# marqo-ai/marqo

Measured on NVIDIA H100. Metric: embeddings/s (open_clip/ViT-L-14 image vectorise, batch 256 per GPU), higher is better.
Workload: dtype bf16

## Files before the change

marqo_b200/csrc/attention.cuh:

```cuda
#pragma once
#include <type_traits>

#include "common.cuh"

namespace mb {
namespace attention {

enum Mask { MASK_NONE = 0, MASK_CAUSAL = 1, MASK_KEYLEN = 2 };

constexpr int BQ = 64;

struct RelBias {
    const float* table = nullptr;
    int smax = 0;
};
constexpr int MAX_BIAS_S = 1024;

int launch(const __nv_bfloat16* qkv, __nv_bfloat16* out, int B, int S, int W, int H, int mask, const int32_t* kv_len,
           const RelBias& bias, cudaStream_t stream);

void launch_wgmma_kernel(const __nv_bfloat16* qkv, __nv_bfloat16* out, int B, int S, int W, int H, int hd, int mask,
                         const int32_t* kv_len, const RelBias& bias, cudaStream_t stream);

inline int head_dim(int W, int H) {
    if (H > 0 && W == H * 64) return 64;
    if (H > 0 && W == H * 32) return 32;
    fail(B200_ERR_UNSUPPORTED, "attention: head_dim must be 32 or 64 (width %d, heads %d)", W, H);
}

inline float head_scale_log2e(int hd) { return (hd == 64 ? 0.125f : 0.17677669529663687f) * 1.4426950408889634f; }

template <class F>
void dispatch(int hd, int mask, bool bias, F&& f) {
    if (bias) return f(std::integral_constant<int, 64>{}, std::integral_constant<int, MASK_KEYLEN>{}, std::true_type{});
    const auto with_mask = [&](auto d) {
        if (mask == MASK_NONE)
            f(d, std::integral_constant<int, MASK_NONE>{}, std::false_type{});
        else if (mask == MASK_CAUSAL)
            f(d, std::integral_constant<int, MASK_CAUSAL>{}, std::false_type{});
        else
            f(d, std::integral_constant<int, MASK_KEYLEN>{}, std::false_type{});
    };
    if (hd == 64)
        with_mask(std::integral_constant<int, 64>{});
    else
        with_mask(std::integral_constant<int, 32>{});
}

struct KeyRange {
    int len, nkb;
};
template <int MASK, int BKV>
__device__ __forceinline__ KeyRange key_range(int S, const int32_t* __restrict__ kv_len, int b, int q0) {
    int len = S;
    if (MASK == MASK_KEYLEN) len = min(S, max(kv_len[b], 0));
    int kend = len;
    if (MASK == MASK_CAUSAL) kend = min(len, q0 + BQ);
    return {len, (kend + BKV - 1) / BKV};
}

template <int BKV, int THREADS>
__device__ __forceinline__ void stage_bias_band(float* band, const float* __restrict__ rel_bias, int smax, int h, int q0,
                                                int nkb) {
    const float* row = rel_bias + (size_t)h * (2 * smax - 1);
    for (int t = threadIdx.x; t < nkb * BKV + BQ; t += THREADS) {
        const int idx = t - (q0 + BQ - 1) + smax - 1;
        band[t] = idx >= 0 && idx < 2 * smax - 1 ? __ldg(row + idx) : 0.f;
    }
}

template <int MASK, bool BIAS>
struct OnlineSoftmax {
    int qrow[2];
    int q0;
    int len;
    float scale_log2e;
    const float* band;
    float row_sum[2] = {0.f, 0.f};
    float row_max[2] = {-INFINITY, -INFINITY};

    template <int NS, int NO>
    __device__ __forceinline__ void update(float (&s)[NS], float (&o)[NO], uint32_t (&pa)[NS / 8][4], int key0) {
        const int t = threadIdx.x & 3;
        float mx[2] = {row_max[0], row_max[1]};
#pragma unroll
        for (int i = 0; i < NS / 4; ++i) {
#pragma unroll
            for (int e = 0; e < 4; ++e) {
                const int key = key0 + 8 * i + 2 * t + (e & 1);
                const int rr = e >> 1;
                bool ok = key < len;
                if (MASK == MASK_CAUSAL) ok = ok && key <= qrow[rr];
                float v;
                if constexpr (BIAS)
                    v = ok ? s[4 * i + e] * scale_log2e + band[key - qrow[rr] + (q0 + BQ - 1)] : -INFINITY;
                else
                    v = ok ? s[4 * i + e] * scale_log2e : -INFINITY;
                s[4 * i + e] = v;
                mx[rr] = fmaxf(mx[rr], v);
            }
        }
        float corr[2], msafe[2];
#pragma unroll
        for (int rr = 0; rr < 2; ++rr) {
            mx[rr] = fmaxf(mx[rr], __shfl_xor_sync(0xffffffffu, mx[rr], 1));
            mx[rr] = fmaxf(mx[rr], __shfl_xor_sync(0xffffffffu, mx[rr], 2));
            msafe[rr] = mx[rr] == -INFINITY ? 0.f : mx[rr];
            corr[rr] = exp2f(row_max[rr] - msafe[rr]);
            row_max[rr] = mx[rr];
            row_sum[rr] *= corr[rr];
        }
#pragma unroll
        for (int i = 0; i < NO / 4; ++i) {
            o[4 * i] *= corr[0];
            o[4 * i + 1] *= corr[0];
            o[4 * i + 2] *= corr[1];
            o[4 * i + 3] *= corr[1];
        }
#pragma unroll
        for (int i = 0; i < NS / 4; ++i) {
            const float p0 = exp2f(s[4 * i] - msafe[0]), p1 = exp2f(s[4 * i + 1] - msafe[0]);
            const float p2 = exp2f(s[4 * i + 2] - msafe[1]), p3 = exp2f(s[4 * i + 3] - msafe[1]);
            row_sum[0] += p0 + p1;
            row_sum[1] += p2 + p3;
            pa[i >> 1][(i & 1) * 2] = pack_bf16x2(p0, p1);
            pa[i >> 1][(i & 1) * 2 + 1] = pack_bf16x2(p2, p3);
        }
    }

    __device__ __forceinline__ void finish(float (&inv)[2]) {
#pragma unroll
        for (int rr = 0; rr < 2; ++rr) {
            row_sum[rr] += __shfl_xor_sync(0xffffffffu, row_sum[rr], 1);
            row_sum[rr] += __shfl_xor_sync(0xffffffffu, row_sum[rr], 2);
        }
        inv[0] = row_sum[0] > 0.f ? 1.f / row_sum[0] : 0.f;
        inv[1] = row_sum[1] > 0.f ? 1.f / row_sum[1] : 0.f;
    }
};

}
}
```

marqo_b200/csrc/attention_wgmma.cu:

```cuda
#include <mutex>

#include "attention.cuh"
#include "ptx.cuh"

namespace mb {
namespace attention {

namespace {

constexpr int BKV = 128;
constexpr int KV_STAGES = 2;
constexpr int THREADS = 160;

template <int HD>
struct Tiles {
    static constexpr uint32_t Q_BYTES = BQ * HD * 2;
    static constexpr uint32_t KV_TILE_BYTES = BKV * HD * 2;
    static constexpr uint32_t STAGE_BYTES = 2 * KV_TILE_BYTES;
    static constexpr size_t SMEM_BYTES = Q_BYTES + KV_STAGES * STAGE_BYTES + 1024  + 64 ;
};

template <int HD>
__device__ __forceinline__ uint64_t desc_k(uint32_t smem_addr) {
    if constexpr (HD == 64) return ptx::make_desc_k_sw128(smem_addr);
    else return ptx::make_desc_k_sw64(smem_addr);
}
template <int HD>
__device__ __forceinline__ uint64_t desc_mn(uint32_t smem_addr) {
    if constexpr (HD == 64) return ptx::make_desc_mn_sw128(smem_addr, 0);
    else return ptx::make_desc_mn_sw64(smem_addr, 0);
}

template <int HD>
__device__ __forceinline__ void wgmma_pv(float (&o)[HD / 2], const uint32_t (&a)[4], uint64_t desc_v) {
    if constexpr (HD == 64) ptx::wgmma_m64n64k16_bf16_rs_tb(o, a, desc_v, 1u);
    else ptx::wgmma_m64n32k16_bf16_rs_tb(o, a, desc_v, 1u);
}

inline size_t bias_band_bytes(int S) { return ((size_t)(S + BKV - 1) / BKV * BKV + BQ) * sizeof(float); }

template <int HD, int MASK, bool BIAS>
__global__ void __launch_bounds__(THREADS)
attention_wgmma_kernel(const __grid_constant__ CUtensorMap tmap_q, const __grid_constant__ CUtensorMap tmap_kv,
                       __nv_bfloat16* __restrict__ out, int S, int W, const int32_t* __restrict__ kv_len,
                       float scale_log2e, const float* __restrict__ rel_bias, int bias_smax) {
    constexpr uint32_t Q_BYTES = Tiles<HD>::Q_BYTES;
    constexpr uint32_t KV_TILE_BYTES = Tiles<HD>::KV_TILE_BYTES;
    constexpr uint32_t STAGE_BYTES = Tiles<HD>::STAGE_BYTES;
    extern __shared__ uint8_t smem_raw[];
    uint8_t* smem = reinterpret_cast<uint8_t*>((reinterpret_cast<uintptr_t>(smem_raw) + 1023) & ~uintptr_t(1023));
    uint8_t* sq = smem;
    uint8_t* skv = smem + Q_BYTES;
    uint64_t* full = reinterpret_cast<uint64_t*>(skv + KV_STAGES * STAGE_BYTES);
    uint64_t* empty = full + KV_STAGES;
    uint64_t* qfull = empty + KV_STAGES;

    const int b = blockIdx.z, h = blockIdx.y, q0 = blockIdx.x * BQ;
    const int warp = threadIdx.x >> 5, lane = threadIdx.x & 31;
    const KeyRange kr = key_range<MASK, BKV>(S, kv_len, b, q0);
    const int nkb = kr.nkb;
    const int row0 = b * S;

    if (threadIdx.x == 0) {
        for (int i = 0; i < KV_STAGES; ++i) {
            ptx::mbar_init(&full[i], 1);
            ptx::mbar_init(&empty[i], 4);
        }
        ptx::mbar_init(qfull, 1);
        ptx::fence_barrier_init();
    }
    float* sbias = reinterpret_cast<float*>(reinterpret_cast<uint8_t*>(full) + 64);
    if constexpr (BIAS) stage_bias_band<BKV, THREADS>(sbias, rel_bias, bias_smax, h, q0, nkb);
    __syncthreads();

    if (warp == 4) {
        if (lane == 0 && nkb > 0) {
            ptx::mbar_arrive_expect_tx(qfull, Q_BYTES);
            ptx::tma_load_2d(sq, &tmap_q, qfull, h * HD, row0 + q0, ptx::kEvictFirst);
            for (int j = 0; j < nkb; ++j) {
                const int st = j % KV_STAGES;
                ptx::mbar_wait(&empty[st], ((uint32_t)(j / KV_STAGES) & 1u) ^ 1u);
                ptx::mbar_arrive_expect_tx(&full[st], STAGE_BYTES);
                uint8_t* dst = skv + (size_t)st * STAGE_BYTES;
                ptx::tma_load_2d(dst, &tmap_kv, &full[st], W + h * HD, row0 + j * BKV, ptx::kEvictLast);
                ptx::tma_load_2d(dst + KV_TILE_BYTES, &tmap_kv, &full[st], 2 * W + h * HD, row0 + j * BKV, ptx::kEvictLast);
            }
        }
        return;
    }

    const int g = lane >> 2, t = lane & 3;
    float o[HD / 2];
#pragma unroll
    for (int i = 0; i < HD / 2; ++i) o[i] = 0.f;
    OnlineSoftmax<MASK, BIAS> sm{{q0 + warp * 16 + g, q0 + warp * 16 + g + 8}, q0, kr.len, scale_log2e, sbias};
    if (nkb > 0) ptx::mbar_wait(qfull, 0);
    const uint32_t q_base = ptx::smem_u32(sq);
    for (int j = 0; j < nkb; ++j) {
        const int st = j % KV_STAGES;
        ptx::mbar_wait(&full[st], (uint32_t)(j / KV_STAGES) & 1u);
        const uint32_t k_base = ptx::smem_u32(skv + (size_t)st * STAGE_BYTES);
        const uint32_t v_base = k_base + KV_TILE_BYTES;
        float s[BKV / 2];
        ptx::wgmma_fence();
#pragma unroll
        for (int k = 0; k < HD / 16; ++k)
            ptx::wgmma_m64n128k16_bf16(s, desc_k<HD>(q_base + k * 32), desc_k<HD>(k_base + k * 32), k != 0 ? 1u : 0u);
        ptx::wgmma_commit();
        ptx::wgmma_wait<0>();
        uint32_t pa[BKV / 16][4];
        sm.update(s, o, pa, j * BKV);
        ptx::wgmma_fence();
#pragma unroll
        for (int k = 0; k < BKV / 16; ++k) wgmma_pv<HD>(o, pa[k], desc_mn<HD>(v_base + k * 32 * HD));
        ptx::wgmma_commit();
        ptx::wgmma_wait<0>();
        __syncwarp();
        if (lane == 0) ptx::mbar_arrive(&empty[st]);
    }
    float inv[2];
    sm.finish(inv);
#pragma unroll
    for (int rr = 0; rr < 2; ++rr) {
        if (sm.qrow[rr] >= S) continue;
        __nv_bfloat16* dst = out + ((size_t)row0 + sm.qrow[rr]) * W + h * HD + 2 * t;
#pragma unroll
        for (int i = 0; i < HD / 8; ++i)
            *reinterpret_cast<uint32_t*>(dst + 8 * i) =
                pack_bf16x2(o[4 * i + 2 * rr] * inv[rr], o[4 * i + 2 * rr + 1] * inv[rr]);
    }
}

template <int HD>
void make_tmaps(const __nv_bfloat16* qkv, int B, int S, int W, CUtensorMap& tq, CUtensorMap& tkv) {
    const uint64_t rows = (uint64_t)B * S;
    const CUtensorMapSwizzle swz = HD == 64 ? CU_TENSOR_MAP_SWIZZLE_128B : CU_TENSOR_MAP_SWIZZLE_64B;
    tq = make_tmap_2d(qkv, CU_TENSOR_MAP_DATA_TYPE_BFLOAT16, 2, (uint64_t)3 * W, rows, (uint64_t)3 * W * 2, HD, BQ, swz);
    tkv = make_tmap_2d(qkv, CU_TENSOR_MAP_DATA_TYPE_BFLOAT16, 2, (uint64_t)3 * W, rows, (uint64_t)3 * W * 2, HD, BKV, swz);
}

}

void launch_wgmma_kernel(const __nv_bfloat16* qkv, __nv_bfloat16* out, int B, int S, int W, int H, int hd, int mask,
                         const int32_t* kv_len, const RelBias& bias, cudaStream_t stream) {
    dispatch(hd, mask, bias.table != nullptr, [&](auto d, auto m, auto with_bias) {
        constexpr int HD = decltype(d)::value, MASK = decltype(m)::value;
        constexpr bool BIAS = decltype(with_bias)::value;
        constexpr size_t BASE = Tiles<HD>::SMEM_BYTES;
        static std::once_flag once;
        std::call_once(once, [] {
            MB_CUDA(cudaFuncSetAttribute(attention_wgmma_kernel<HD, MASK, BIAS>,
                                         cudaFuncAttributeMaxDynamicSharedMemorySize,
                                         (int)(BASE + (BIAS ? bias_band_bytes(MAX_BIAS_S) : 0))));
        });
        CUtensorMap tq, tkv;
        make_tmaps<HD>(qkv, B, S, W, tq, tkv);
        attention_wgmma_kernel<HD, MASK, BIAS>
            <<<dim3((S + BQ - 1) / BQ, H, B), THREADS, BASE + (BIAS ? bias_band_bytes(S) : 0), stream>>>(
                tq, tkv, out, S, W, kv_len, head_scale_log2e(HD), bias.table, bias.smax);
    });
}

}
}
```

marqo_b200/csrc/ptx.cuh:

```cuda
#pragma once
#include <cstdint>
#include <cstdio>
#include <cuda.h>
#include <cuda_runtime.h>

namespace ptx {

__device__ __forceinline__ uint32_t smem_u32(const void* p) {
    return static_cast<uint32_t>(__cvta_generic_to_shared(p));
}

__device__ __forceinline__ void st_shared_u32(uint32_t addr, uint32_t v) {
    asm volatile("st.shared.b32 [%0], %1;" ::"r"(addr), "r"(v) : "memory");
}
__device__ __forceinline__ void st_shared_f32x2(uint32_t addr, float x, float y) {
    asm volatile("st.shared.v2.f32 [%0], {%1, %2};" ::"r"(addr), "f"(x), "f"(y) : "memory");
}
__device__ __forceinline__ uint32_t ld_shared_u32(uint32_t addr) {
    uint32_t v;
    asm volatile("ld.shared.b32 %0, [%1];" : "=r"(v) : "r"(addr) : "memory");
    return v;
}
__device__ __forceinline__ float2 ld_shared_f32x2(uint32_t addr) {
    float2 v;
    asm volatile("ld.shared.v2.f32 {%0, %1}, [%2];" : "=f"(v.x), "=f"(v.y) : "r"(addr) : "memory");
    return v;
}

__device__ __forceinline__ uint32_t lane_id() {
    uint32_t l;
    asm volatile("mov.u32 %0, %%laneid;" : "=r"(l));
    return l;
}

__device__ __forceinline__ uint64_t globaltimer_ns() {
    uint64_t t;
    asm volatile("mov.u64 %0, %%globaltimer;" : "=l"(t));
    return t;
}

__device__ __forceinline__ bool elect_one() {
    uint32_t pred;
    asm volatile(
        "{\n"
        ".reg .pred p;\n"
        "elect.sync _|p, 0xffffffff;\n"
        "selp.u32 %0, 1, 0, p;\n"
        "}\n"
        : "=r"(pred));
    return pred != 0;
}

__device__ __forceinline__ void mbar_init(uint64_t* bar, uint32_t count) {
    asm volatile("mbarrier.init.shared::cta.b64 [%0], %1;" ::"r"(smem_u32(bar)), "r"(count) : "memory");
}
__device__ __forceinline__ void fence_barrier_init() {
    asm volatile("fence.mbarrier_init.release.cluster;" ::: "memory");
}
__device__ __forceinline__ void fence_proxy_async_smem() {
    asm volatile("fence.proxy.async.shared::cta;" ::: "memory");
}
__device__ __forceinline__ void mbar_arrive_expect_tx(uint64_t* bar, uint32_t bytes) {
    asm volatile("mbarrier.arrive.expect_tx.shared::cta.b64 _, [%0], %1;" ::"r"(smem_u32(bar)), "r"(bytes)
                 : "memory");
}
__device__ __forceinline__ void mbar_arrive(uint64_t* bar) {
    asm volatile("mbarrier.arrive.shared::cta.b64 _, [%0];" ::"r"(smem_u32(bar)) : "memory");
}
__device__ __forceinline__ bool mbar_try_wait(uint64_t* bar, uint32_t parity) {
    uint32_t ok;
    asm volatile(
        "{\n"
        ".reg .pred p;\n"
        "mbarrier.try_wait.parity.shared::cta.b64 p, [%1], %2;\n"
        "selp.u32 %0, 1, 0, p;\n"
        "}\n"
        : "=r"(ok)
        : "r"(smem_u32(bar)), "r"(parity)
        : "memory");
    return ok != 0;
}
__device__ __forceinline__ void mbar_wait(uint64_t* bar, uint32_t parity) {
    if (mbar_try_wait(bar, parity)) return;
    uint64_t t0 = globaltimer_ns();
    uint32_t spins = 0;
    while (!mbar_try_wait(bar, parity)) {
        if ((++spins & 0x3ff) == 0 && globaltimer_ns() - t0 > 4000000000ull) __trap();
    }
}

constexpr uint64_t kEvictNormal = 0x1000000000000000ull;
constexpr uint64_t kEvictFirst = 0x12F0000000000000ull;
constexpr uint64_t kEvictLast = 0x14F0000000000000ull;

__device__ __forceinline__ void prefetch_tmap(const CUtensorMap* tmap) {
    asm volatile("prefetch.tensormap [%0];" ::"l"(reinterpret_cast<uint64_t>(tmap)) : "memory");
}

__device__ __forceinline__ void tma_load_2d(void* smem_dst, const CUtensorMap* tmap, uint64_t* bar, int32_t c0,
                                            int32_t c1, uint64_t cache_hint) {
    asm volatile(
        "cp.async.bulk.tensor.2d.shared::cluster.global.tile.mbarrier::complete_tx::bytes.L2::cache_hint"
        " [%0], [%1, {%3, %4}], [%2], %5;"
        ::"r"(smem_u32(smem_dst)), "l"(reinterpret_cast<uint64_t>(tmap)), "r"(smem_u32(bar)), "r"(c0), "r"(c1),
        "l"(cache_hint)
        : "memory");
}

__device__ __forceinline__ void tma_prefetch_l2_2d(const CUtensorMap* tmap, int32_t c0, int32_t c1) {
    asm volatile("cp.async.bulk.prefetch.tensor.2d.L2.global.tile [%0, {%1, %2}];" ::"l"(reinterpret_cast<uint64_t>(tmap)),
                 "r"(c0), "r"(c1)
                 : "memory");
}

__device__ __forceinline__ void tma_store_2d(const CUtensorMap* tmap, const void* smem_src, int32_t c0, int32_t c1) {
    asm volatile("cp.async.bulk.tensor.2d.global.shared::cta.tile.bulk_group [%0, {%2, %3}], [%1];" ::"l"(
                     reinterpret_cast<uint64_t>(tmap)),
                 "r"(smem_u32(smem_src)), "r"(c0), "r"(c1)
                 : "memory");
}
__device__ __forceinline__ void tma_store_commit() { asm volatile("cp.async.bulk.commit_group;" ::: "memory"); }
template <int N>
__device__ __forceinline__ void tma_store_wait_read() {
    asm volatile("cp.async.bulk.wait_group.read %0;" ::"n"(N) : "memory");
}
template <int N>
__device__ __forceinline__ void tma_store_wait() {
    asm volatile("cp.async.bulk.wait_group %0;" ::"n"(N) : "memory");
}

__device__ __forceinline__ uint64_t make_desc_k_sw128(uint32_t smem_addr) {
    uint64_t d = 0;
    d |= static_cast<uint64_t>((smem_addr & 0x3FFFF) >> 4);
    d |= static_cast<uint64_t>(1) << 16;
    d |= static_cast<uint64_t>(1024 >> 4) << 32;
    d |= static_cast<uint64_t>(1) << 62;
    return d;
}

__device__ __forceinline__ uint64_t make_desc_mn_sw128(uint32_t smem_addr, uint32_t lbo_bytes) {
    uint64_t d = 0;
    d |= static_cast<uint64_t>((smem_addr & 0x3FFFF) >> 4);
    d |= static_cast<uint64_t>((lbo_bytes >> 4) & 0x3FFF) << 16;
    d |= static_cast<uint64_t>(1024 >> 4) << 32;
    d |= static_cast<uint64_t>(1) << 62;
    return d;
}

__device__ __forceinline__ uint64_t make_desc_k_sw64(uint32_t smem_addr) {
    uint64_t d = 0;
    d |= static_cast<uint64_t>((smem_addr & 0x3FFFF) >> 4);
    d |= static_cast<uint64_t>(1) << 16;
    d |= static_cast<uint64_t>(512 >> 4) << 32;
    d |= static_cast<uint64_t>(2) << 62;
    return d;
}

__device__ __forceinline__ uint64_t make_desc_mn_sw64(uint32_t smem_addr, uint32_t lbo_bytes) {
    uint64_t d = 0;
    d |= static_cast<uint64_t>((smem_addr & 0x3FFFF) >> 4);
    d |= static_cast<uint64_t>((lbo_bytes >> 4) & 0x3FFF) << 16;
    d |= static_cast<uint64_t>(512 >> 4) << 32;
    d |= static_cast<uint64_t>(2) << 62;
    return d;
}

__device__ __forceinline__ void wgmma_fence() { asm volatile("wgmma.fence.sync.aligned;" ::: "memory"); }
__device__ __forceinline__ void wgmma_commit() { asm volatile("wgmma.commit_group.sync.aligned;" ::: "memory"); }
template <int N>
__device__ __forceinline__ void wgmma_wait() {
    asm volatile("wgmma.wait_group.sync.aligned %0;" ::"n"(N) : "memory");
}

__device__ __forceinline__ void wgmma_m64n128k16_f16(float (&d)[64], uint64_t desc_a, uint64_t desc_b, uint32_t scale_d) {
    asm volatile(
        "{\n"
        ".reg .pred p;\n"
        "setp.ne.b32 p, %66, 0;\n"
        "wgmma.mma_async.sync.aligned.m64n128k16.f32.f16.f16 "
        "{"
        "%0, %1, %2, %3, %4, %5, %6, %7, %8, %9, %10, %11, %12, %13, %14, %15, "
        "%16, %17, %18, %19, %20, %21, %22, %23, %24, %25, %26, %27, %28, %29, %30, %31, "
        "%32, %33, %34, %35, %36, %37, %38, %39, %40, %41, %42, %43, %44, %45, %46, %47, "
        "%48, %49, %50, %51, %52, %53, %54, %55, %56, %57, %58, %59, %60, %61, %62, %63"
        "}, %64, %65, p, 1, 1, 0, 0;\n"
        "}\n"
        : "+f"(d[0]), "+f"(d[1]), "+f"(d[2]), "+f"(d[3]), "+f"(d[4]), "+f"(d[5]), "+f"(d[6]), "+f"(d[7]),
          "+f"(d[8]), "+f"(d[9]), "+f"(d[10]), "+f"(d[11]), "+f"(d[12]), "+f"(d[13]), "+f"(d[14]), "+f"(d[15]),
          "+f"(d[16]), "+f"(d[17]), "+f"(d[18]), "+f"(d[19]), "+f"(d[20]), "+f"(d[21]), "+f"(d[22]), "+f"(d[23]),
          "+f"(d[24]), "+f"(d[25]), "+f"(d[26]), "+f"(d[27]), "+f"(d[28]), "+f"(d[29]), "+f"(d[30]), "+f"(d[31]),
          "+f"(d[32]), "+f"(d[33]), "+f"(d[34]), "+f"(d[35]), "+f"(d[36]), "+f"(d[37]), "+f"(d[38]), "+f"(d[39]),
          "+f"(d[40]), "+f"(d[41]), "+f"(d[42]), "+f"(d[43]), "+f"(d[44]), "+f"(d[45]), "+f"(d[46]), "+f"(d[47]),
          "+f"(d[48]), "+f"(d[49]), "+f"(d[50]), "+f"(d[51]), "+f"(d[52]), "+f"(d[53]), "+f"(d[54]), "+f"(d[55]),
          "+f"(d[56]), "+f"(d[57]), "+f"(d[58]), "+f"(d[59]), "+f"(d[60]), "+f"(d[61]), "+f"(d[62]), "+f"(d[63])
        : "l"(desc_a), "l"(desc_b), "r"(scale_d));
}
__device__ __forceinline__ void wgmma_m64n128k16_bf16(float (&d)[64], uint64_t desc_a, uint64_t desc_b, uint32_t scale_d) {
    asm volatile(
        "{\n"
        ".reg .pred p;\n"
        "setp.ne.b32 p, %66, 0;\n"
        "wgmma.mma_async.sync.aligned.m64n128k16.f32.bf16.bf16 "
        "{"
        "%0, %1, %2, %3, %4, %5, %6, %7, %8, %9, %10, %11, %12, %13, %14, %15, "
        "%16, %17, %18, %19, %20, %21, %22, %23, %24, %25, %26, %27, %28, %29, %30, %31, "
        "%32, %33, %34, %35, %36, %37, %38, %39, %40, %41, %42, %43, %44, %45, %46, %47, "
        "%48, %49, %50, %51, %52, %53, %54, %55, %56, %57, %58, %59, %60, %61, %62, %63"
        "}, %64, %65, p, 1, 1, 0, 0;\n"
        "}\n"
        : "+f"(d[0]), "+f"(d[1]), "+f"(d[2]), "+f"(d[3]), "+f"(d[4]), "+f"(d[5]), "+f"(d[6]), "+f"(d[7]),
          "+f"(d[8]), "+f"(d[9]), "+f"(d[10]), "+f"(d[11]), "+f"(d[12]), "+f"(d[13]), "+f"(d[14]), "+f"(d[15]),
          "+f"(d[16]), "+f"(d[17]), "+f"(d[18]), "+f"(d[19]), "+f"(d[20]), "+f"(d[21]), "+f"(d[22]), "+f"(d[23]),
          "+f"(d[24]), "+f"(d[25]), "+f"(d[26]), "+f"(d[27]), "+f"(d[28]), "+f"(d[29]), "+f"(d[30]), "+f"(d[31]),
          "+f"(d[32]), "+f"(d[33]), "+f"(d[34]), "+f"(d[35]), "+f"(d[36]), "+f"(d[37]), "+f"(d[38]), "+f"(d[39]),
          "+f"(d[40]), "+f"(d[41]), "+f"(d[42]), "+f"(d[43]), "+f"(d[44]), "+f"(d[45]), "+f"(d[46]), "+f"(d[47]),
          "+f"(d[48]), "+f"(d[49]), "+f"(d[50]), "+f"(d[51]), "+f"(d[52]), "+f"(d[53]), "+f"(d[54]), "+f"(d[55]),
          "+f"(d[56]), "+f"(d[57]), "+f"(d[58]), "+f"(d[59]), "+f"(d[60]), "+f"(d[61]), "+f"(d[62]), "+f"(d[63])
        : "l"(desc_a), "l"(desc_b), "r"(scale_d));
}
__device__ __forceinline__ void wgmma_m64n256k16_bf16(float (&d)[128], uint64_t desc_a, uint64_t desc_b, uint32_t scale_d) {
    asm volatile(
        "{\n"
        ".reg .pred p;\n"
        "setp.ne.b32 p, %130, 0;\n"
        "wgmma.mma_async.sync.aligned.m64n256k16.f32.bf16.bf16 "
        "{"
        "%0, %1, %2, %3, %4, %5, %6, %7, %8, %9, %10, %11, %12, %13, %14, %15, "
        "%16, %17, %18, %19, %20, %21, %22, %23, %24, %25, %26, %27, %28, %29, %30, %31, "
        "%32, %33, %34, %35, %36, %37, %38, %39, %40, %41, %42, %43, %44, %45, %46, %47, "
        "%48, %49, %50, %51, %52, %53, %54, %55, %56, %57, %58, %59, %60, %61, %62, %63, "
        "%64, %65, %66, %67, %68, %69, %70, %71, %72, %73, %74, %75, %76, %77, %78, %79, "
        "%80, %81, %82, %83, %84, %85, %86, %87, %88, %89, %90, %91, %92, %93, %94, %95, "
        "%96, %97, %98, %99, %100, %101, %102, %103, %104, %105, %106, %107, %108, %109, %110, %111, "
        "%112, %113, %114, %115, %116, %117, %118, %119, %120, %121, %122, %123, %124, %125, %126, %127"
        "}, %128, %129, p, 1, 1, 0, 0;\n"
        "}\n"
        : "+f"(d[0]), "+f"(d[1]), "+f"(d[2]), "+f"(d[3]), "+f"(d[4]), "+f"(d[5]), "+f"(d[6]), "+f"(d[7]),
          "+f"(d[8]), "+f"(d[9]), "+f"(d[10]), "+f"(d[11]), "+f"(d[12]), "+f"(d[13]), "+f"(d[14]), "+f"(d[15]),
          "+f"(d[16]), "+f"(d[17]), "+f"(d[18]), "+f"(d[19]), "+f"(d[20]), "+f"(d[21]), "+f"(d[22]), "+f"(d[23]),
          "+f"(d[24]), "+f"(d[25]), "+f"(d[26]), "+f"(d[27]), "+f"(d[28]), "+f"(d[29]), "+f"(d[30]), "+f"(d[31]),
          "+f"(d[32]), "+f"(d[33]), "+f"(d[34]), "+f"(d[35]), "+f"(d[36]), "+f"(d[37]), "+f"(d[38]), "+f"(d[39]),
          "+f"(d[40]), "+f"(d[41]), "+f"(d[42]), "+f"(d[43]), "+f"(d[44]), "+f"(d[45]), "+f"(d[46]), "+f"(d[47]),
          "+f"(d[48]), "+f"(d[49]), "+f"(d[50]), "+f"(d[51]), "+f"(d[52]), "+f"(d[53]), "+f"(d[54]), "+f"(d[55]),
          "+f"(d[56]), "+f"(d[57]), "+f"(d[58]), "+f"(d[59]), "+f"(d[60]), "+f"(d[61]), "+f"(d[62]), "+f"(d[63]),
          "+f"(d[64]), "+f"(d[65]), "+f"(d[66]), "+f"(d[67]), "+f"(d[68]), "+f"(d[69]), "+f"(d[70]), "+f"(d[71]),
          "+f"(d[72]), "+f"(d[73]), "+f"(d[74]), "+f"(d[75]), "+f"(d[76]), "+f"(d[77]), "+f"(d[78]), "+f"(d[79]),
          "+f"(d[80]), "+f"(d[81]), "+f"(d[82]), "+f"(d[83]), "+f"(d[84]), "+f"(d[85]), "+f"(d[86]), "+f"(d[87]),
          "+f"(d[88]), "+f"(d[89]), "+f"(d[90]), "+f"(d[91]), "+f"(d[92]), "+f"(d[93]), "+f"(d[94]), "+f"(d[95]),
          "+f"(d[96]), "+f"(d[97]), "+f"(d[98]), "+f"(d[99]), "+f"(d[100]), "+f"(d[101]), "+f"(d[102]), "+f"(d[103]),
          "+f"(d[104]), "+f"(d[105]), "+f"(d[106]), "+f"(d[107]), "+f"(d[108]), "+f"(d[109]), "+f"(d[110]), "+f"(d[111]),
          "+f"(d[112]), "+f"(d[113]), "+f"(d[114]), "+f"(d[115]), "+f"(d[116]), "+f"(d[117]), "+f"(d[118]), "+f"(d[119]),
          "+f"(d[120]), "+f"(d[121]), "+f"(d[122]), "+f"(d[123]), "+f"(d[124]), "+f"(d[125]), "+f"(d[126]), "+f"(d[127])
        : "l"(desc_a), "l"(desc_b), "r"(scale_d));
}
__device__ __forceinline__ void wgmma_m64n64k16_bf16_rs_tb(float (&d)[32], const uint32_t (&a)[4], uint64_t desc_b, uint32_t scale_d) {
    asm volatile(
        "{\n"
        ".reg .pred p;\n"
        "setp.ne.b32 p, %37, 0;\n"
        "wgmma.mma_async.sync.aligned.m64n64k16.f32.bf16.bf16 "
        "{"
        "%0, %1, %2, %3, %4, %5, %6, %7, %8, %9, %10, %11, %12, %13, %14, %15, "
        "%16, %17, %18, %19, %20, %21, %22, %23, %24, %25, %26, %27, %28, %29, %30, %31"
        "}, {%32, %33, %34, %35}, %36, p, 1, 1, 1;\n"
        "}\n"
        : "+f"(d[0]), "+f"(d[1]), "+f"(d[2]), "+f"(d[3]), "+f"(d[4]), "+f"(d[5]), "+f"(d[6]), "+f"(d[7]),
          "+f"(d[8]), "+f"(d[9]), "+f"(d[10]), "+f"(d[11]), "+f"(d[12]), "+f"(d[13]), "+f"(d[14]), "+f"(d[15]),
          "+f"(d[16]), "+f"(d[17]), "+f"(d[18]), "+f"(d[19]), "+f"(d[20]), "+f"(d[21]), "+f"(d[22]), "+f"(d[23]),
          "+f"(d[24]), "+f"(d[25]), "+f"(d[26]), "+f"(d[27]), "+f"(d[28]), "+f"(d[29]), "+f"(d[30]), "+f"(d[31])
        : "r"(a[0]), "r"(a[1]), "r"(a[2]), "r"(a[3]), "l"(desc_b), "r"(scale_d));
}
__device__ __forceinline__ void wgmma_m64n32k16_bf16_rs_tb(float (&d)[16], const uint32_t (&a)[4], uint64_t desc_b, uint32_t scale_d) {
    asm volatile(
        "{\n"
        ".reg .pred p;\n"
        "setp.ne.b32 p, %21, 0;\n"
        "wgmma.mma_async.sync.aligned.m64n32k16.f32.bf16.bf16 "
        "{"
        "%0, %1, %2, %3, %4, %5, %6, %7, %8, %9, %10, %11, %12, %13, %14, %15"
        "}, {%16, %17, %18, %19}, %20, p, 1, 1, 1;\n"
        "}\n"
        : "+f"(d[0]), "+f"(d[1]), "+f"(d[2]), "+f"(d[3]), "+f"(d[4]), "+f"(d[5]), "+f"(d[6]), "+f"(d[7]),
          "+f"(d[8]), "+f"(d[9]), "+f"(d[10]), "+f"(d[11]), "+f"(d[12]), "+f"(d[13]), "+f"(d[14]), "+f"(d[15])
        : "r"(a[0]), "r"(a[1]), "r"(a[2]), "r"(a[3]), "l"(desc_b), "r"(scale_d));
}
template <int REGS>
__device__ __forceinline__ void setmaxnreg_inc() {
    asm volatile("setmaxnreg.inc.sync.aligned.u32 %0;" ::"n"(REGS));
}
template <int REGS>
__device__ __forceinline__ void setmaxnreg_dec() {
    asm volatile("setmaxnreg.dec.sync.aligned.u32 %0;" ::"n"(REGS));
}

template <int ID, int COUNT>
__device__ __forceinline__ void bar_sync() {
    asm volatile("bar.sync %0, %1;" ::"n"(ID), "n"(COUNT) : "memory");
}

}
```

Baseline: 2788.

## Narrow final key tile in wgmma attention and skip masking on full tiles

```diff
diff --git a/marqo_b200/csrc/attention.cuh b/marqo_b200/csrc/attention.cuh
--- a/marqo_b200/csrc/attention.cuh
+++ b/marqo_b200/csrc/attention.cuh
@@ -48,7 +48,7 @@
 }
 
 struct KeyRange {
-    int len, nkb;
+    int len, nkb, kend;
 };
 template <int MASK, int BKV>
 __device__ __forceinline__ KeyRange key_range(int S, const int32_t* __restrict__ kv_len, int b, int q0) {
@@ -56,7 +56,7 @@
     if (MASK == MASK_KEYLEN) len = min(S, max(kv_len[b], 0));
     int kend = len;
     if (MASK == MASK_CAUSAL) kend = min(len, q0 + BQ);
-    return {len, (kend + BKV - 1) / BKV};
+    return {len, (kend + BKV - 1) / BKV, kend};
 }
 
 template <int BKV, int THREADS>
@@ -79,7 +79,7 @@
     float row_sum[2] = {0.f, 0.f};
     float row_max[2] = {-INFINITY, -INFINITY};
 
-    template <int NS, int NO>
+    template <bool FULL = false, int NS, int NO>
     __device__ __forceinline__ void update(float (&s)[NS], float (&o)[NO], uint32_t (&pa)[NS / 8][4], int key0) {
         const int t = threadIdx.x & 3;
         float mx[2] = {row_max[0], row_max[1]};
@@ -89,8 +89,8 @@
             for (int e = 0; e < 4; ++e) {
                 const int key = key0 + 8 * i + 2 * t + (e & 1);
                 const int rr = e >> 1;
-                bool ok = key < len;
-                if (MASK == MASK_CAUSAL) ok = ok && key <= qrow[rr];
+                bool ok = FULL || key < len;
+                if (!FULL && MASK == MASK_CAUSAL) ok = ok && key <= qrow[rr];
                 float v;
                 if constexpr (BIAS)
                     v = ok ? s[4 * i + e] * scale_log2e + band[key - qrow[rr] + (q0 + BQ - 1)] : -INFINITY;
diff --git a/marqo_b200/csrc/attention_wgmma.cu b/marqo_b200/csrc/attention_wgmma.cu
--- a/marqo_b200/csrc/attention_wgmma.cu
+++ b/marqo_b200/csrc/attention_wgmma.cu
@@ -35,6 +35,41 @@
 __device__ __forceinline__ void wgmma_pv(float (&o)[HD / 2], const uint32_t (&a)[4], uint64_t desc_v) {
     if constexpr (HD == 64) ptx::wgmma_m64n64k16_bf16_rs_tb(o, a, desc_v, 1u);
     else ptx::wgmma_m64n32k16_bf16_rs_tb(o, a, desc_v, 1u);
+}
+
+template <int NW>
+__device__ __forceinline__ void wgmma_qk(float (&s)[NW / 2], uint64_t desc_q, uint64_t desc_kk, uint32_t scale_d) {
+    static_assert(NW == 16 || NW == 32 || NW == 64 || NW == 128, "key tile widths");
+    if constexpr (NW == 128) ptx::wgmma_m64n128k16_bf16(s, desc_q, desc_kk, scale_d);
+    else if constexpr (NW == 64) ptx::wgmma_m64n64k16_bf16(s, desc_q, desc_kk, scale_d);
+    else if constexpr (NW == 32) ptx::wgmma_m64n32k16_bf16(s, desc_q, desc_kk, scale_d);
+    else ptx::wgmma_m64n16k16_bf16(s, desc_q, desc_kk, scale_d);
+}
+
+template <int HD, int NW, bool FULL, int MASK, bool BIAS>
+__device__ __forceinline__ void key_tile(OnlineSoftmax<MASK, BIAS>& sm, float (&o)[HD / 2], uint32_t q_base,
+                                         uint32_t k_base, uint32_t v_base, int key0, bool live) {
+    float s[NW / 2];
+    ptx::wgmma_fence();
+#pragma unroll
+    for (int k = 0; k < HD / 16; ++k)
+        wgmma_qk<NW>(s, desc_k<HD>(q_base + k * 32), desc_k<HD>(k_base + k * 32), k != 0 ? 1u : 0u);
+    ptx::wgmma_commit();
+    ptx::wgmma_wait<0>();
+    uint32_t pa[NW / 16][4];
+    if (live) {
+        sm.template update<FULL>(s, o, pa, key0);
+    } else {
+#pragma unroll
+        for (int k = 0; k < NW / 16; ++k)
+#pragma unroll
+            for (int c = 0; c < 4; ++c) asm volatile("mov.b32 %0, 0;" : "=r"(pa[k][c]));
+    }
+    ptx::wgmma_fence();
+#pragma unroll
+    for (int k = 0; k < NW / 16; ++k) wgmma_pv<HD>(o, pa[k], desc_mn<HD>(v_base + k * 32 * HD));
+    ptx::wgmma_commit();
+    ptx::wgmma_wait<0>();
 }
 
 inline size_t bias_band_bytes(int S) { return ((size_t)(S + BKV - 1) / BKV * BKV + BQ) * sizeof(float); }
@@ -58,7 +93,8 @@
     const int b = blockIdx.z, h = blockIdx.y, q0 = blockIdx.x * BQ;
     const int warp = threadIdx.x >> 5, lane = threadIdx.x & 31;
     const KeyRange kr = key_range<MASK, BKV>(S, kv_len, b, q0);
-    const int nkb = kr.nkb;
+    const int nkb = __shfl_sync(0xffffffffu, kr.nkb, 0);
+    const int tail = __shfl_sync(0xffffffffu, kr.kend - (kr.nkb - 1) * BKV, 0);
     const int row0 = b * S;
 
     if (threadIdx.x == 0) {
@@ -96,25 +132,24 @@
     OnlineSoftmax<MASK, BIAS> sm{{q0 + warp * 16 + g, q0 + warp * 16 + g + 8}, q0, kr.len, scale_log2e, sbias};
     if (nkb > 0) ptx::mbar_wait(qfull, 0);
     const uint32_t q_base = ptx::smem_u32(sq);
+    const bool live = q0 + warp * 16 < S;
+    static_assert(BKV % BQ == 0, "interior key tiles end on a query-block edge");
+    const bool last_full = tail == BKV && MASK != MASK_CAUSAL;
     for (int j = 0; j < nkb; ++j) {
         const int st = j % KV_STAGES;
         ptx::mbar_wait(&full[st], (uint32_t)(j / KV_STAGES) & 1u);
         const uint32_t k_base = ptx::smem_u32(skv + (size_t)st * STAGE_BYTES);
         const uint32_t v_base = k_base + KV_TILE_BYTES;
-        float s[BKV / 2];
-        ptx::wgmma_fence();
-#pragma unroll
-        for (int k = 0; k < HD / 16; ++k)
-            ptx::wgmma_m64n128k16_bf16(s, desc_k<HD>(q_base + k * 32), desc_k<HD>(k_base + k * 32), k != 0 ? 1u : 0u);
-        ptx::wgmma_commit();
-        ptx::wgmma_wait<0>();
-        uint32_t pa[BKV / 16][4];
-        sm.update(s, o, pa, j * BKV);
-        ptx::wgmma_fence();
-#pragma unroll
-        for (int k = 0; k < BKV / 16; ++k) wgmma_pv<HD>(o, pa[k], desc_mn<HD>(v_base + k * 32 * HD));
-        ptx::wgmma_commit();
-        ptx::wgmma_wait<0>();
+        if (j < nkb - 1 || last_full)
+            key_tile<HD, BKV, true>(sm, o, q_base, k_base, v_base, j * BKV, live);
+        else if (tail <= 16)
+            key_tile<HD, 16, false>(sm, o, q_base, k_base, v_base, j * BKV, live);
+        else if (tail <= 32)
+            key_tile<HD, 32, false>(sm, o, q_base, k_base, v_base, j * BKV, live);
+        else if (tail <= 64)
+            key_tile<HD, 64, false>(sm, o, q_base, k_base, v_base, j * BKV, live);
+        else
+            key_tile<HD, BKV, false>(sm, o, q_base, k_base, v_base, j * BKV, live);
         __syncwarp();
         if (lane == 0) ptx::mbar_arrive(&empty[st]);
     }
diff --git a/marqo_b200/csrc/ptx.cuh b/marqo_b200/csrc/ptx.cuh
--- a/marqo_b200/csrc/ptx.cuh
+++ b/marqo_b200/csrc/ptx.cuh
@@ -216,6 +216,50 @@
           "+f"(d[40]), "+f"(d[41]), "+f"(d[42]), "+f"(d[43]), "+f"(d[44]), "+f"(d[45]), "+f"(d[46]), "+f"(d[47]),
           "+f"(d[48]), "+f"(d[49]), "+f"(d[50]), "+f"(d[51]), "+f"(d[52]), "+f"(d[53]), "+f"(d[54]), "+f"(d[55]),
           "+f"(d[56]), "+f"(d[57]), "+f"(d[58]), "+f"(d[59]), "+f"(d[60]), "+f"(d[61]), "+f"(d[62]), "+f"(d[63])
+        : "l"(desc_a), "l"(desc_b), "r"(scale_d));
+}
+__device__ __forceinline__ void wgmma_m64n64k16_bf16(float (&d)[32], uint64_t desc_a, uint64_t desc_b, uint32_t scale_d) {
+    asm volatile(
+        "{\n"
+        ".reg .pred p;\n"
+        "setp.ne.b32 p, %34, 0;\n"
+        "wgmma.mma_async.sync.aligned.m64n64k16.f32.bf16.bf16 "
+        "{"
+        "%0, %1, %2, %3, %4, %5, %6, %7, %8, %9, %10, %11, %12, %13, %14, %15, "
+        "%16, %17, %18, %19, %20, %21, %22, %23, %24, %25, %26, %27, %28, %29, %30, %31"
+        "}, %32, %33, p, 1, 1, 0, 0;\n"
+        "}\n"
+        : "+f"(d[0]), "+f"(d[1]), "+f"(d[2]), "+f"(d[3]), "+f"(d[4]), "+f"(d[5]), "+f"(d[6]), "+f"(d[7]),
+          "+f"(d[8]), "+f"(d[9]), "+f"(d[10]), "+f"(d[11]), "+f"(d[12]), "+f"(d[13]), "+f"(d[14]), "+f"(d[15]),
+          "+f"(d[16]), "+f"(d[17]), "+f"(d[18]), "+f"(d[19]), "+f"(d[20]), "+f"(d[21]), "+f"(d[22]), "+f"(d[23]),
+          "+f"(d[24]), "+f"(d[25]), "+f"(d[26]), "+f"(d[27]), "+f"(d[28]), "+f"(d[29]), "+f"(d[30]), "+f"(d[31])
+        : "l"(desc_a), "l"(desc_b), "r"(scale_d));
+}
+__device__ __forceinline__ void wgmma_m64n32k16_bf16(float (&d)[16], uint64_t desc_a, uint64_t desc_b, uint32_t scale_d) {
+    asm volatile(
+        "{\n"
+        ".reg .pred p;\n"
+        "setp.ne.b32 p, %18, 0;\n"
+        "wgmma.mma_async.sync.aligned.m64n32k16.f32.bf16.bf16 "
+        "{"
+        "%0, %1, %2, %3, %4, %5, %6, %7, %8, %9, %10, %11, %12, %13, %14, %15"
+        "}, %16, %17, p, 1, 1, 0, 0;\n"
+        "}\n"
+        : "+f"(d[0]), "+f"(d[1]), "+f"(d[2]), "+f"(d[3]), "+f"(d[4]), "+f"(d[5]), "+f"(d[6]), "+f"(d[7]),
+          "+f"(d[8]), "+f"(d[9]), "+f"(d[10]), "+f"(d[11]), "+f"(d[12]), "+f"(d[13]), "+f"(d[14]), "+f"(d[15])
+        : "l"(desc_a), "l"(desc_b), "r"(scale_d));
+}
+__device__ __forceinline__ void wgmma_m64n16k16_bf16(float (&d)[8], uint64_t desc_a, uint64_t desc_b, uint32_t scale_d) {
+    asm volatile(
+        "{\n"
+        ".reg .pred p;\n"
+        "setp.ne.b32 p, %10, 0;\n"
+        "wgmma.mma_async.sync.aligned.m64n16k16.f32.bf16.bf16 "
+        "{"
+        "%0, %1, %2, %3, %4, %5, %6, %7"
+        "}, %8, %9, p, 1, 1, 0, 0;\n"
+        "}\n"
+        : "+f"(d[0]), "+f"(d[1]), "+f"(d[2]), "+f"(d[3]), "+f"(d[4]), "+f"(d[5]), "+f"(d[6]), "+f"(d[7])
         : "l"(desc_a), "l"(desc_b), "r"(scale_d));
 }
 __device__ __forceinline__ void wgmma_m64n256k16_bf16(float (&d)[128], uint64_t desc_a, uint64_t desc_b, uint32_t scale_d) {
```

Measured after the change: 2849, median of 6. 1.02x the previous value.
